# strasdat/ScaViSLAM

Measured on AMD Instinct MI355X. Metric: stereo frames/sec + DWO Schur ms @ 50 KF / 20k pts, higher is better.
Workload: dtype u8/int32 (FAST, ZNSSD), f32+f64 (dense tracking), f64 (Schur); 1 GPU

## Files before the change

scavislam_amd/csrc/motion.hip:

```cpp
#include "common.h"
#include "gate.h"
#include "lm6.h"
#include <algorithm>

namespace {

__device__ __forceinline__ void cloud_TQ(const double (&T)[12], const svs_cam &cam, double (&TQ)[16]) {
  double Ti[12];
#pragma unroll
  for (int r = 0; r < 3; ++r)
#pragma unroll
    for (int c = 0; c < 3; ++c) Ti[4 * r + c] = T[4 * c + r];
#pragma unroll
  for (int r = 0; r < 3; ++r) Ti[4 * r + 3] = -(Ti[4 * r] * T[3] + Ti[4 * r + 1] * T[7] + Ti[4 * r + 2] * T[11]);
  const double Q[16] = {1, 0, 0, -cam.cx, 0, 1, 0, -cam.cy, 0, 0, 0, cam.f, 0, 0, 1.0 / cam.b, 0};
#pragma unroll
  for (int r = 0; r < 4; ++r)
#pragma unroll
    for (int c = 0; c < 4; ++c) {
      double s = 0;
#pragma unroll
      for (int k = 0; k < 4; ++k) { double tik = r < 3 ? Ti[4 * r + k] : (k == 3 ? 1.0 : 0.0); s += tik * Q[4 * k + c]; }
      TQ[4 * r + c] = s;
    }
}
__device__ __forceinline__ void cloud_sample(const float *__restrict__ disp, int ds, int cw, int level, const double (&TQ)[16], int i, float *__restrict__ cloud) {
  const int u = i % cw, v = i / cw;
  const double inv_factor = 1.0 / (double)(1 << level);
  const float d = (float)(disp[(size_t)((v * 4) << level) * ds + ((u * 4) << level)] * inv_factor);
  float4 o;
  if (d <= 0) o = make_float4(0.f, 0.f, 0.f, -1.f);
  else {
    const double q[4] = {(double)(u * 4), (double)(v * 4), (double)d, 1.0};
    double r[4];
#pragma unroll
    for (int k = 0; k < 4; ++k) r[k] = TQ[4 * k] * q[0] + TQ[4 * k + 1] * q[1] + TQ[4 * k + 2] * q[2] + TQ[4 * k + 3] * q[3];
    o = make_float4((float)(r[0] / r[3]), (float)(r[1] / r[3]), (float)(r[2] / r[3]), 1.f);
  }
  reinterpret_cast<float4 *>(cloud)[i] = o;
}
__global__ __launch_bounds__(256) void pointcloud_cpu_sem_kernel(const float *__restrict__ disp, int ds, size_t disp_b, svs_cam cam,
                                                                 int level, const double *__restrict__ Tarr,
                                                                 float *__restrict__ cloud, size_t cloud_b) {
  const int slot = blockIdx.y;
  const int cw = cam.w / 4, ch = cam.h / 4;
  const int i = blockIdx.x * 256 + threadIdx.x;
  if (i >= cw * ch) return;
  double T[12], TQ[16];
#pragma unroll
  for (int k = 0; k < 12; ++k) T[k] = Tarr[(size_t)slot * 12 + k];
  cloud_TQ(T, cam, TQ);
  cloud_sample(disp + slot * disp_b, ds, cw, level, TQ, i, cloud + slot * cloud_b);
}

struct CloudLevels { svs_cam cam[3]; float *cloud[3]; size_t cloud_b[3]; int blocks[3]; };
__global__ __launch_bounds__(256) void pointcloud_cpu_sem_levels_kernel(const float *__restrict__ disp, int ds, size_t disp_b, CloudLevels Q, const double *__restrict__ Tarr) {
  const int slot = blockIdx.y;
  int bx = blockIdx.x, level = 0;
  if (bx >= Q.blocks[0]) { bx -= Q.blocks[0]; level = 1; if (bx >= Q.blocks[1]) { bx -= Q.blocks[1]; level = 2; } }
  const svs_cam cam = level == 0 ? Q.cam[0] : (level == 1 ? Q.cam[1] : Q.cam[2]);
  float *cloud = level == 0 ? Q.cloud[0] : (level == 1 ? Q.cloud[1] : Q.cloud[2]);
  const size_t cloud_b = level == 0 ? Q.cloud_b[0] : (level == 1 ? Q.cloud_b[1] : Q.cloud_b[2]);
  const int cw = cam.w / 4, ch = cam.h / 4;
  const int i = bx * 256 + threadIdx.x;
  if (i >= cw * ch) return;
  double T[12], TQ[16];
#pragma unroll
  for (int k = 0; k < 12; ++k) T[k] = Tarr[(size_t)slot * 12 + k];
  cloud_TQ(T, cam, TQ);
  cloud_sample(disp + slot * disp_b, ds, cw, level, TQ, i, cloud + slot * cloud_b);
}

}

int svs_pointcloud_cpu_sem_levels(svs_ctx *ctx, const float *d_disp, int disp_stride, size_t disp_bstride, const svs_cam *cams, const double *d_T, float *const *d_cloud,
                                  const size_t *cloud_bstride, int batch) {
  SVS_REQUIRE(ctx, ctx && d_disp && cams && d_T && d_cloud && cloud_bstride && batch >= 1);
  SVS_DEVICE(ctx);
  CloudLevels Q;
  int total = 0;
  for (int l = 0; l < 3; ++l) {
    SVS_REQUIRE(ctx, cams[l].w % 4 == 0 && cams[l].h % 4 == 0 && d_cloud[l]);
    Q.cam[l] = cams[l]; Q.cloud[l] = d_cloud[l]; Q.cloud_b[l] = cloud_bstride[l];
    Q.blocks[l] = div_up((cams[l].w / 4) * (cams[l].h / 4), 256);
    total += Q.blocks[l];
  }
  hipLaunchKernelGGL(pointcloud_cpu_sem_levels_kernel, dim3(total, batch), dim3(256), 0, ctx->stream, d_disp, disp_stride, disp_bstride, Q, d_T);
  SVS_LAUNCH_CHECK(ctx);
  return SVS_OK;
}

extern "C" int svs_pointcloud_cpu_sem(svs_ctx *ctx, const float *d_disp, int disp_stride, size_t disp_bstride,
                                      const svs_cam *cam, int level, const double *d_T, float *d_cloud,
                                      size_t cloud_bstride, int batch) {
  SVS_REQUIRE(ctx, ctx && d_disp && cam && d_T && d_cloud && level >= 0 && level < 3 && batch >= 1);
  SVS_DEVICE(ctx);
  SVS_REQUIRE(ctx, cam->w % 4 == 0 && cam->h % 4 == 0);
  int n = (cam->w / 4) * (cam->h / 4);
  hipLaunchKernelGGL(pointcloud_cpu_sem_kernel, dim3(div_up(n, 256), batch), dim3(256), 0, ctx->stream, d_disp, disp_stride,
                     disp_bstride, *cam, level, d_T, d_cloud, cloud_bstride);
  SVS_LAUNCH_CHECK(ctx);
  return SVS_OK;
}

namespace {

__device__ __forceinline__ double mo_kernel(double delta, double b) {
  const double a = fabs(delta);
  return a < b ? delta * delta : 2 * b * a - b * b;
}
__device__ __forceinline__ double mo_weighted_sq(double *f, int robust, double b) {
  if (robust) {
    const double nrm = fmax(1e-10, sqrt(f[0] * f[0] + f[1] * f[1] + f[2] * f[2]));
    const double w = sqrt(mo_kernel(nrm, b)) / nrm;
    f[0] *= w; f[1] *= w; f[2] *= w;
  }
  return f[0] * f[0] + f[1] * f[1] + f[2] * f[2];
}

constexpr int MO_THREADS = 256;
template <int N>
__device__ __forceinline__ void mo_reduce(double (&v)[N], int n_sum, double *s_red) {
  const int lane = threadIdx.x & 63, wave = threadIdx.x >> 6;
#pragma unroll
  for (int k = 0; k < N; ++k) {
    double x = v[k];
#pragma unroll
    for (int o = 32; o > 0; o >>= 1) { const double y = __shfl_xor(x, o, 64); x = k < n_sum ? x + y : fmax(x, y); }
    if (lane == 0) s_red[wave * N + k] = x;
  }
  __syncthreads();
  if (threadIdx.x < N) {
    const int k = threadIdx.x;
    double x = s_red[k];
    for (int w = 1; w < MO_THREADS / 64; ++w) x = k < n_sum ? x + s_red[w * N + k] : fmax(x, s_red[w * N + k]);
    s_red[(MO_THREADS / 64) * N + k] = x;
  }
  __syncthreads();
#pragma unroll
  for (int k = 0; k < N; ++k) v[k] = s_red[(MO_THREADS / 64) * N + k];
  __syncthreads();
}

__global__ __launch_bounds__(MO_THREADS) void motion_only_kernel(const svs_match_result *__restrict__ res, int n, size_t res_bstride, svs_cam cam,
                                                                 svs_pose_opt_params prm, double *__restrict__ T_io, svs_pose_opt_stats *__restrict__ stats) {
  __shared__ double s_red[(MO_THREADS / 64 + 1) * 28];
  __shared__ double s_T[12], s_Tn[12], s_B[6];
  const int tid = threadIdx.x, slot = blockIdx.x;
  res += (size_t)slot * res_bstride;
  if (tid < 12) s_T[tid] = T_io[12 * slot + tid];
  __syncthreads();
  double chi2, max_err, mu, nu = 2;
  int num_obs;
  {
    double v[4] = {0, 0, 0, 0};
    for (int i = tid; i < n; i += MO_THREADS) {
      if (res[i].status != 0) continue;
      double f[3], J[18];
      mo_residual<true>(s_T, res[i], cam, f, J);
#pragma unroll
      for (int c = 0; c < 6; ++c) v[3] = fmax(v[3], fabs(J[c] * J[c] + J[6 + c] * J[6 + c] + J[12 + c] * J[12 + c]));
      v[0] += mo_weighted_sq(f, prm.robust_kernel, prm.kernel_param);
      v[1] += 1.0;
      v[2] = fmax(v[2], fmax(fabs(f[0]), fmax(fabs(f[1]), fabs(f[2]))));
    }
    mo_reduce<4>(v, 2, s_red);
    chi2 = v[0]; num_obs = (int)v[1]; max_err = v[2];
    mu = prm.initial_mu == -1 ? prm.tau * v[3] : prm.initial_mu;
  }
  const double initial_chi2 = chi2;
  int status = num_obs == 0 ? 1 : (num_obs < prm.min_obs ? 3 : 0), trial = 0;
  bool stop = status != 0;
  for (int ig = 0; ig < prm.num_iter && !stop; ++ig) {
    double rho = 0;
    do {
      double v[27];
#pragma unroll
      for (int k = 0; k < 27; ++k) v[k] = 0;
      for (int i = tid; i < n; i += MO_THREADS) {
        if (res[i].status != 0) continue;
        double f[3], J[18];
        mo_residual<true>(s_T, res[i], cam, f, J);
        mo_weighted_sq(f, prm.robust_kernel, prm.kernel_param);
        int k = 0;
#pragma unroll
        for (int r = 0; r < 6; ++r) {
#pragma unroll
          for (int c = r; c < 6; ++c) v[k++] += J[r] * J[c] + J[6 + r] * J[6 + c] + J[12 + r] * J[12 + c];
          v[21 + r] += J[r] * f[0] + J[6 + r] * f[1] + J[12 + r] * f[2];
        }
      }
      mo_reduce<27>(v, 27, s_red);
      if (tid == 0) {
        double A[36], B[6], delta[6];
        int k = 0;
        for (int r = 0; r < 6; ++r)
          for (int c = r; c < 6; ++c) { A[6 * r + c] = A[6 * c + r] = v[k++]; }
        for (int r = 0; r < 6; ++r) { A[7 * r] += mu; B[r] = -v[21 + r]; s_B[r] = B[r]; }
        d_solve6(A, B, delta);
        double Tn[12];
        d_se3_exp_mul(delta, s_T, Tn);
        for (int i = 0; i < 12; ++i) s_Tn[i] = Tn[i];
      }
      __syncthreads();
      double w[2] = {0, 0};
      for (int i = tid; i < n; i += MO_THREADS) {
        if (res[i].status != 0) continue;
        double f[3];
        mo_residual<false>(s_Tn, res[i], cam, f, nullptr);
        w[0] += mo_weighted_sq(f, prm.robust_kernel, prm.kernel_param);
        w[1] = fmax(w[1], fmax(fabs(f[0]), fmax(fabs(f[1]), fabs(f[2]))));
      }
      mo_reduce<2>(w, 1, s_red);
      const double new_chi2 = w[0];
      if (isnan(new_chi2)) { status = 2; stop = true; break; }
      rho = chi2 - new_chi2;
      if (rho > 0) {
        if (tid < 12) s_T[tid] = s_Tn[tid];
        chi2 = new_chi2; max_err = w[1];
        double bm = -1;
        for (int c = 0; c < 6; ++c) bm = fmax(bm, fabs(s_B[c]));
        stop = bm <= 1e-10;
        const double q = 2 * rho - 1, sc = 1 - q * q * q;
        mu *= fmax(1. / 3., sc);
        nu = 2.; trial = 0;
      } else {
        mu *= nu; nu *= 2.; ++trial;
        if (trial == 5) stop = true;
      }
      __syncthreads();
    } while (!(rho > 0 || stop));
  }
  if (tid < 12) T_io[12 * slot + tid] = s_T[tid];
  if (tid == 0) {
    svs_pose_opt_stats st;
    st.initial_chi2 = initial_chi2; st.chi2 = chi2; st.max_err = max_err; st.num_obs = num_obs; st.status = status;
    stats[slot] = st;
  }
}

constexpr int MO2_THREADS = 256, MO2_RC = 6, MO2_WAVES = MO2_THREADS / 64;
struct MoObs { double o[3], q[3]; };

template <bool FIRST, bool JAC = true>
__device__ __forceinline__ void mo2_terms(const double (&T)[12], const MoObs &ob, const svs_cam &cam, int robust, double kb, double (&x)[32], double &max_err,
                                          double &max_diag) {
  static_assert(JAC || !FIRST, "the first sweep needs the Jacobian");
  const double *q = ob.q;
  const double X = T[0] * q[0] + T[1] * q[1] + T[2] * q[2] + T[3];
  const double Y = T[4] * q[0] + T[5] * q[1] + T[6] * q[2] + T[7];
  const double Z = T[8] * q[0] + T[9] * q[1] + T[10] * q[2] + T[11];
  const double fl = cam.f, iz = 1.0 / Z, fiz = fl * iz, Xb = X - cam.b;
  double f0 = ob.o[0] - (X * fiz + cam.cx), f1 = ob.o[1] - (Y * fiz + cam.cy), f2 = ob.o[2] - (Xb * fiz + cam.cx);
  const double A = -fiz, C = fiz * X * iz, D = fiz * Y * iz, E = fiz * Xb * iz;
  const double a3 = Y * C, a4 = Z * A - X * C, a5 = -Y * A;
  const double b3 = Y * D - Z * A, b4 = -X * D, b5 = X * A;
  const double c3 = Y * E, c4 = Z * A - X * E;
  if (FIRST) {
    const double AA = A * A;
    double m = fmax(AA + AA, AA);
    m = fmax(m, C * C + D * D + E * E);
    m = fmax(m, a3 * a3 + b3 * b3 + c3 * c3);
    m = fmax(m, a4 * a4 + b4 * b4 + c4 * c4);
    m = fmax(m, a5 * a5 + b5 * b5 + a5 * a5);
    max_diag = fmax(max_diag, m);
  }
  const double ss = f0 * f0 + f1 * f1 + f2 * f2;
  double chi = ss;
  if (robust) {
    const double nrm = fmax(1e-10, sqrt(ss));
    if (nrm >= kb) {
      const double k = 2 * kb * nrm - kb * kb, w = sqrt(k) / nrm;
      f0 *= w; f1 *= w; f2 *= w;
      chi = f0 * f0 + f1 * f1 + f2 * f2;
    }
  }
  x[27] += chi;
  max_err = fmax(max_err, fmax(fabs(f0), fmax(fabs(f1), fabs(f2))));
  if constexpr (!JAC) return;
  x[0] += A * A + A * A;          x[1] += 0.0;                     x[2] += A * C + A * E;
  x[3] += A * a3 + A * c3;        x[4] += A * a4 + A * c4;         x[5] += A * a5 + A * a5;
  x[6] += A * A;                  x[7] += A * D;                   x[8] += A * b3;
  x[9] += A * b4;                 x[10] += A * b5;
  x[11] += C * C + D * D + E * E; x[12] += C * a3 + D * b3 + E * c3; x[13] += C * a4 + D * b4 + E * c4;
  x[14] += C * a5 + D * b5 + E * a5;
  x[15] += a3 * a3 + b3 * b3 + c3 * c3; x[16] += a3 * a4 + b3 * b4 + c3 * c4; x[17] += a3 * a5 + b3 * b5 + c3 * a5;
  x[18] += a4 * a4 + b4 * b4 + c4 * c4; x[19] += a4 * a5 + b4 * b5 + c4 * a5;
  x[20] += a5 * a5 + b5 * b5 + a5 * a5;
  x[21] += A * f0 + A * f2;       x[22] += A * f1;                 x[23] += C * f0 + D * f1 + E * f2;
  x[24] += a3 * f0 + b3 * f1 + c3 * f2; x[25] += a4 * f0 + b4 * f1 + c4 * f2; x[26] += a5 * f0 + b5 * f1 + a5 * f2;
}
__device__ __forceinline__ int mo2_id(int lane) { return ((lane & 1) << 4) | ((lane & 2) << 2) | (lane & 4) | ((lane & 8) >> 2) | ((lane & 16) >> 4); }
__device__ __forceinline__ double mo2_wave_reduce(double (&x)[32]) {
  const int lane = threadIdx.x & 63;
#pragma unroll
  for (int step = 0; step < 5; ++step) {
    const int half = 16 >> step, bit = 1 << step;
    const bool up = (lane & bit) != 0;
#pragma unroll
    for (int k = 0; k < half; ++k) {
      double lo = x[k], hi = x[k + half];
      asm volatile("" : "+v"(lo), "+v"(hi));
      const double send = up ? lo : hi;
      const double keep = up ? hi : lo;
      x[k] = keep + __shfl_xor(send, bit, 64);
    }
  }
  return x[0] + __shfl_xor(x[0], 32, 64);
}

template <bool FIRST>
__device__ __forceinline__ void mo2_sweep(const double (&T)[12], const MoObs (&ob)[MO2_RC], int n_ok, const int *s_idx, const svs_match_result *__restrict__ res,
                                          const svs_cam &cam, int robust, double kb, double (*s_part)[32]) {
  const int tid = threadIdx.x, lane = tid & 63, wave = tid >> 6;
  double x[32];
#pragma unroll
  for (int i = 0; i < 32; ++i) x[i] = 0.0;
  double me = 0.0, md = 0.0;
#pragma unroll
  for (int k = 0; k < MO2_RC; ++k)
    if (tid + k * MO2_THREADS < n_ok) mo2_terms<FIRST>(T, ob[k], cam, robust, kb, x, me, md);
  for (int j = tid + MO2_RC * MO2_THREADS; j < n_ok; j += MO2_THREADS) {
    const svs_match_result &r = res[s_idx[j]];
    MoObs t;
#pragma unroll
    for (int c = 0; c < 3; ++c) { t.o[c] = r.obs[c]; t.q[c] = r.xyz_actkey[c]; }
    mo2_terms<FIRST>(T, t, cam, robust, kb, x, me, md);
  }
  const double v = mo2_wave_reduce(x);
#pragma unroll
  for (int o = 32; o > 0; o >>= 1) { me = fmax(me, __shfl_xor(me, o, 64)); if (FIRST) md = fmax(md, __shfl_xor(md, o, 64)); }
  const int id = mo2_id(lane);
  if (lane < 32 && id < 28) s_part[wave][id] = v;
  if (lane == 0) { s_part[wave][28] = me; s_part[wave][29] = md; }
}

__device__ __forceinline__ void mo2_sweep_chi2(const double (&T)[12], const MoObs (&ob)[MO2_RC], int n_ok, const int *s_idx, const svs_match_result *__restrict__ res,
                                               const svs_cam &cam, int robust, double kb, double (*s_part)[32]) {
  const int tid = threadIdx.x, lane = tid & 63, wave = tid >> 6;
  double x[32];
  x[27] = 0.0;
  double me = 0.0, md = 0.0;
#pragma unroll
  for (int k = 0; k < MO2_RC; ++k)
    if (tid + k * MO2_THREADS < n_ok) mo2_terms<false, false>(T, ob[k], cam, robust, kb, x, me, md);
  for (int j = tid + MO2_RC * MO2_THREADS; j < n_ok; j += MO2_THREADS) {
    const svs_match_result &r = res[s_idx[j]];
    MoObs t;
#pragma unroll
    for (int c = 0; c < 3; ++c) { t.o[c] = r.obs[c]; t.q[c] = r.xyz_actkey[c]; }
    mo2_terms<false, false>(T, t, cam, robust, kb, x, me, md);
  }
  double v = x[27];
#pragma unroll
  for (int o = 1; o <= 32; o <<= 1) v += __shfl_xor(v, o, 64);
#pragma unroll
  for (int o = 32; o > 0; o >>= 1) me = fmax(me, __shfl_xor(me, o, 64));
  if (lane == 0) { s_part[wave][27] = v; s_part[wave][28] = me; }
}

__device__ __forceinline__ void gate_stream(const svs_match_result *__restrict__ res, const svs_candidate_point *__restrict__ pts, int n, int n_new, const svs_cam &cam,
                                            const double (&T)[12], float mre, svs_gated_point *__restrict__ out, svs_point_stats *__restrict__ st, int tid, int *s_cnt,
                                            double *s_sum) {
  if (tid < 18) s_cnt[tid] = 0;
  __syncthreads();
  const int half_w = (int)(cam.w * 0.5), half_h = (int)(cam.h * 0.5);
  const float third = (float)(1. / 3.);
  const int third_w = (int)(cam.w * third), third_h = (int)(cam.h * third);
  const int tt_w = (int)(cam.w * 2 * third), tt_h = (int)(cam.h * 2 * third);
  double len = 0;
  for (int i = tid; i < n && tid < 256; i += 256) {
    svs_gated_point g{};
    if (res[i].status == 0) {
      atomicAdd(&s_cnt[17], 1);
      double d[3];
      mo_residual<false>(T, res[i], cam, d, nullptr);
      const int level = pts[i].anchor_level;
      const int factor = 1 << level;
      if (SVS_GATE_PASSES(d, factor, mre)) {
        const double *uvu = res[i].obs, *q = res[i].xyz_actkey;
        const int i2 = uvu[0] < half_w ? 0 : 1, j2 = uvu[1] < half_h ? 0 : 1;
        const int i3 = uvu[0] < third_w ? 0 : (uvu[0] < tt_w ? 1 : 2), j3 = uvu[1] < third_h ? 0 : (uvu[1] < tt_h ? 1 : 2);
        atomicAdd(&s_cnt[i2 * 2 + j2], 1);
        atomicAdd(&s_cnt[4 + i3 * 3 + j3], 1);
        atomicAdd(&s_cnt[13 + level], 1);
        atomicAdd(&s_cnt[16], 1);
        const double inv = 1.0 / (double)factor;
        g.accepted = 1;
        g.is_new = i < n_new ? 1 : 0;
        g.uv_pyr[0] = uvu[0] * inv; g.uv_pyr[1] = uvu[1] * inv;
        g.curkey_uv_pyr[0] = (q[0] / q[2] * cam.f + cam.cx) * inv;
        g.curkey_uv_pyr[1] = (q[1] / q[2] * cam.f + cam.cy) * inv;
        const double dx = g.uv_pyr[0] - g.curkey_uv_pyr[0], dy = g.uv_pyr[1] - g.curkey_uv_pyr[1];
        len += sqrt(dx * dx + dy * dy);
      }
    }
    out[i] = g;
  }
#pragma unroll
  for (int o = 32; o > 0; o >>= 1) len += __shfl_xor(len, o, 64);
  if ((tid & 63) == 0 && tid < 256) s_sum[tid >> 6] = len;
  __syncthreads();
  if (tid < 4) st->num_points_grid2x2[tid] = s_cnt[tid];
  else if (tid < 13) st->num_points_grid3x3[tid - 4] = s_cnt[tid];
  else if (tid < 16) st->num_matched_points[tid - 13] = s_cnt[tid];
  else if (tid == 16) st->num_track_points = s_cnt[16];
  else if (tid == 17) st->num_obs = s_cnt[17];
  else if (tid == 18) { st->pad_[0] = st->pad_[1] = 0; st->sum_track_length = (s_sum[0] + s_sum[1]) + (s_sum[2] + s_sum[3]); }
}
using MoTail = svs_mo_tail;
template <bool TAIL>
__global__ __launch_bounds__(MO2_THREADS) void motion_only_fused_kernel(const svs_match_result *__restrict__ res, int n, size_t res_bstride, svs_cam cam,
                                                                        svs_pose_opt_params prm, double *__restrict__ T_io,
                                                                        svs_pose_opt_stats *__restrict__ stats, MoTail Q, int spec) {
  extern __shared__ int s_idx[];
  __shared__ double s_part[MO2_WAVES][32];
  __shared__ double s_Tn[12], s_Tc[12];
  __shared__ int s_wcnt[8][MO2_WAVES];
  __shared__ int s_conv;
  const int tid = threadIdx.x, lane = tid & 63, wave = tid >> 6, slot = TAIL && Q.order ? (Q.order[blockIdx.x] >> 4) : (int)blockIdx.x;
  res += (size_t)slot * res_bstride;
  int n_ok = 0;
  for (int base = 0; base < n; base += 8 * MO2_THREADS) {
    int st[8];
#pragma unroll
    for (int c = 0; c < 8; ++c) { const int i = base + c * MO2_THREADS + tid; st[c] = i < n ? res[i].status : 1; }
    unsigned long long m[8];
#pragma unroll
    for (int c = 0; c < 8; ++c) { m[c] = __ballot(st[c] == 0); if (lane == 0) s_wcnt[c][wave] = __popcll(m[c]); }
    __syncthreads();
#pragma unroll
    for (int c = 0; c < 8; ++c) {
      int off = n_ok, tot = 0;
#pragma unroll
      for (int w = 0; w < MO2_WAVES; ++w) { const int k = s_wcnt[c][w]; off += w < wave ? k : 0; tot += k; }
      if (st[c] == 0) s_idx[off + __popcll(m[c] & ((1ull << lane) - 1ull))] = base + c * MO2_THREADS + tid;
      n_ok += tot;
    }
    __syncthreads();
  }
  MoObs ob[MO2_RC];
#pragma unroll
  for (int k = 0; k < MO2_RC; ++k) {
    const int j = tid + k * MO2_THREADS;
    if (j < n_ok) {
      const svs_match_result &r = res[s_idx[j]];
#pragma unroll
      for (int c = 0; c < 3; ++c) { ob[k].o[c] = r.obs[c]; ob[k].q[c] = r.xyz_actkey[c]; }
    }
  }
  auto total = [&](int id) { double s = s_part[0][id]; for (int w = 1; w < MO2_WAVES; ++w) s += s_part[w][id]; return s; };
  auto total_max = [&](int id) { double s = s_part[0][id]; for (int w = 1; w < MO2_WAVES; ++w) s = fmax(s, s_part[w][id]); return s; };
  auto uniform_pose = [&](const double *p, double (&T)[12]) {
#pragma unroll
    for (int i = 0; i < 12; ++i) {
      const double v = p[i];
      T[i] = __hiloint2double(__builtin_amdgcn_readfirstlane(__double2hiint(v)), __builtin_amdgcn_readfirstlane(__double2loint(v)));
    }
  };
  double Tn[12];
  uniform_pose(T_io + 12 * slot, Tn);
  if (tid < 12) s_Tc[tid] = T_io[12 * slot + tid];
  mo2_sweep<true>(Tn, ob, n_ok, s_idx, res, cam, prm.robust_kernel, prm.kernel_param, s_part);
  __syncthreads();
  const int num_obs = n_ok;
  double chi2 = total(27), max_err = total_max(28), mu = prm.initial_mu == -1 ? prm.tau * total_max(29) : prm.initial_mu, nu = 2;
  const double initial_chi2 = chi2;
  int status = num_obs == 0 ? 1 : (num_obs < prm.min_obs ? 3 : 0), trial = 0;
  bool stop = status != 0;
  double col[6] = {0, 0, 0, 0, 0, 0};
  auto load_system = [&]() {
    if (wave == 0 && lane < 7) {
#pragma unroll
      for (int r = 0; r < 6; ++r) {
        const int a = r < lane ? r : lane, b = r < lane ? lane : r;
        col[r] = lane < 6 ? total(a * (13 - a) / 2 + (b - a)) : -total(21 + r);
      }
    }
  };
  load_system();
  for (int ig = 0; ig < prm.num_iter && !stop; ++ig) {
    double rho = 0;
    do {
      if (wave == 0) {
        double a[6], bmax = 0, delta[6];
#pragma unroll
        for (int r = 0; r < 6; ++r) a[r] = col[r] + (r == lane ? mu : 0.0);
#pragma unroll
        for (int r = 0; r < 6; ++r) bmax = fmax(bmax, fabs(mo2_bcast(col[r], 6)));
        wave_solve6(a, delta);
        double Tc[12], Tx[12];
#pragma unroll
        for (int i = 0; i < 12; ++i) Tc[i] = s_Tc[i];
        mo2_exp_mul(delta, Tc, Tx);
        if (lane < 12) {
          double v = Tx[0];
#pragma unroll
          for (int i = 1; i < 12; ++i) v = lane == i ? Tx[i] : v;
          s_Tn[lane] = v;
        }
        if (lane == 0) s_conv = bmax <= 1e-10 ? 1 : 0;
      }
      __syncthreads();
      uniform_pose(s_Tn, Tn);
      const int conv = s_conv;
      const bool lean = spec != 0 && trial >= 1;
      if (lean) mo2_sweep_chi2(Tn, ob, n_ok, s_idx, res, cam, prm.robust_kernel, prm.kernel_param, s_part);
      else mo2_sweep<false>(Tn, ob, n_ok, s_idx, res, cam, prm.robust_kernel, prm.kernel_param, s_part);
      __syncthreads();
      const double new_chi2 = total(27), new_max = total_max(28);
      if (isnan(new_chi2)) { status = 2; stop = true; break; }
      rho = chi2 - new_chi2;
      if (rho > 0 && lean) {
        __syncthreads();
        mo2_sweep<false>(Tn, ob, n_ok, s_idx, res, cam, prm.robust_kernel, prm.kernel_param, s_part);
        __syncthreads();
      }
      if (rho > 0) {
        if (tid < 12) s_Tc[tid] = s_Tn[tid];
        chi2 = new_chi2; max_err = new_max;
        load_system();
        stop = conv != 0;
        const double q = 2 * rho - 1, sc = 1 - q * q * q;
        mu *= fmax(1. / 3., sc);
        nu = 2.; trial = 0;
      } else {
        mu *= nu; nu *= 2.; ++trial;
        if (trial == 5) stop = true;
      }
    } while (!(rho > 0 || stop));
  }
  if (tid < 12) T_io[12 * slot + tid] = s_Tc[tid];
  if (tid == 0) {
    svs_pose_opt_stats st;
    st.initial_chi2 = initial_chi2; st.chi2 = chi2; st.max_err = max_err; st.num_obs = num_obs; st.status = status;
    stats[slot] = st;
  }
  if constexpr (TAIL) {
    __shared__ int s_gcnt[18];
    __shared__ double s_gsum[4];
    __syncthreads();
    double T[12];
#pragma unroll
    for (int i = 0; i < 12; ++i) T[i] = s_Tc[i];
    gate_stream(res, Q.pts + slot * Q.pts_b, n, Q.n_new[slot], cam, T, Q.mre, Q.gated + slot * Q.gated_b, Q.ptstats + slot, tid, s_gcnt, s_gsum);
#pragma unroll 1
    for (int l = 0; l < 3; ++l) {
      double TQ[16];
      cloud_TQ(T, Q.cams[l], TQ);
      const int cw = Q.cams[l].w / 4, n_px = cw * (Q.cams[l].h / 4);
      const float *disp = Q.disp + slot * Q.disp_b;
      float *cloud = Q.cloud[l] + slot * Q.cloud_b[l];
      for (int i = tid; i < n_px; i += MO2_THREADS) cloud_sample(disp, Q.ds, cw, l, TQ, i, cloud);
    }
  }
}

}
namespace {
__global__ __launch_bounds__(256) void gate_matched_kernel(const svs_match_result *__restrict__ res, const svs_candidate_point *__restrict__ pts, int n,
                                                           size_t res_b, size_t pts_b, int n_new, const int32_t *__restrict__ n_new_arr, svs_cam cam,
                                                           const double *__restrict__ Tarr, float mre, svs_gated_point *__restrict__ out, size_t out_b,
                                                           svs_point_stats *__restrict__ stats) {
  __shared__ int s_cnt[18];
  __shared__ double s_sum[4];
  const int tid = threadIdx.x, slot = blockIdx.x;
  if (n_new_arr) n_new = n_new_arr[slot];
  double T[12];
#pragma unroll
  for (int k = 0; k < 12; ++k) T[k] = Tarr[12 * slot + k];
  gate_stream(res + slot * res_b, pts + slot * pts_b, n, n_new, cam, T, mre, out + slot * out_b, stats + slot, tid, s_cnt, s_sum);
}
}

extern "C" int svs_process_matched_points(svs_ctx *ctx, const svs_match_result *d_results, const svs_candidate_point *d_pts, int n,
                                          size_t res_bstride, size_t pts_bstride, int n_new_records, const svs_cam *cam, const double *d_T,
                                          float max_reproj_error, svs_gated_point *d_gated, size_t gated_bstride, svs_point_stats *d_stats,
                                          int batch) {
  SVS_REQUIRE(ctx, ctx && cam && d_T && d_stats && batch >= 1 && n >= 0 && (n == 0 || (d_results && d_pts && d_gated)));
  SVS_DEVICE(ctx);
  hipLaunchKernelGGL(gate_matched_kernel, dim3(batch), dim3(256), 0, ctx->stream, d_results, d_pts, n, res_bstride, pts_bstride, n_new_records,
                     (const int32_t *)nullptr, *cam, d_T, max_reproj_error, d_gated, gated_bstride, d_stats);
  SVS_LAUNCH_CHECK(ctx);
  return SVS_OK;
}
int svs_process_matched_points_dev(svs_ctx *ctx, const svs_match_result *d_results, const svs_candidate_point *d_pts, int n, size_t res_bstride,
                                   size_t pts_bstride, const int32_t *d_n_new_records, const svs_cam *cam, const double *d_T, float max_reproj_error,
                                   svs_gated_point *d_gated, size_t gated_bstride, svs_point_stats *d_stats, int batch) {
  SVS_REQUIRE(ctx, ctx && cam && d_T && d_stats && d_n_new_records && batch >= 1 && n >= 0 && (n == 0 || (d_results && d_pts && d_gated)));
  SVS_DEVICE(ctx);
  hipLaunchKernelGGL(gate_matched_kernel, dim3(batch), dim3(256), 0, ctx->stream, d_results, d_pts, n, res_bstride, pts_bstride, 0, d_n_new_records, *cam, d_T,
                     max_reproj_error, d_gated, gated_bstride, d_stats);
  SVS_LAUNCH_CHECK(ctx);
  return SVS_OK;
}

int svs_motion_only_gate_cloud(svs_ctx *ctx, const svs_match_result *d_results, int n, size_t res_bstride, const svs_cam *cam, const svs_pose_opt_params *prm,
                               double *d_T_io, svs_pose_opt_stats *d_stats, const svs_mo_tail *tail, int batch) {
  SVS_REQUIRE(ctx, ctx && cam && prm && d_T_io && d_stats && tail && batch >= 1 && n >= 1 && d_results);
  SVS_DEVICE(ctx);
  if ((size_t)n * sizeof(int) > 48 * 1024 || ctx->mo_legacy) return SVS_ERR_UNSUPPORTED;
  for (int l = 0; l < 3; ++l) SVS_REQUIRE(ctx, tail->cams[l].w % 4 == 0 && tail->cams[l].h % 4 == 0 && tail->cloud[l]);
  hipLaunchKernelGGL(motion_only_fused_kernel<true>, dim3(batch), dim3(MO2_THREADS), (size_t)n * sizeof(int), ctx->stream, d_results, n, res_bstride, *cam, *prm, d_T_io,
                     d_stats, *tail, ctx->mo_spec);
  SVS_LAUNCH_CHECK(ctx);
  return SVS_OK;
}

extern "C" int svs_motion_only(svs_ctx *ctx, const svs_match_result *d_results, int n, size_t res_bstride, const svs_cam *cam,
                               const svs_pose_opt_params *prm, double *d_T_io, svs_pose_opt_stats *d_stats, int batch) {
  SVS_REQUIRE(ctx, ctx && cam && prm && d_T_io && d_stats && batch >= 1 && n >= 0 && (n == 0 || d_results));
  SVS_DEVICE(ctx);
  if ((size_t)n * sizeof(int) <= 48 * 1024 && !ctx->mo_legacy)
    hipLaunchKernelGGL(motion_only_fused_kernel<false>, dim3(batch), dim3(MO2_THREADS), (size_t)std::max(n, 1) * sizeof(int), ctx->stream, d_results, n, res_bstride, *cam,
                       *prm, d_T_io, d_stats, MoTail{}, ctx->mo_spec);
  else
    hipLaunchKernelGGL(motion_only_kernel, dim3(batch), dim3(MO_THREADS), 0, ctx->stream, d_results, n, res_bstride, *cam, *prm, d_T_io, d_stats);
  SVS_LAUNCH_CHECK(ctx);
  return SVS_OK;
}
```

Measured before the change: 218,700 frames/s.

## Stage overflow observations in LDS and batch loads in gate and cloud loops

Observations beyond the six register-cached ones per thread are now staged once into shared memory, up to 512 of them. Each LM sweep then reads them from LDS instead of re-gathering them through the index list from global memory. The gating loop and the point-cloud tail loop are restructured to issue several independent global loads (8 and 16 per lane) before computing, which exposes memory-level parallelism. The status-scan load is also clamped so it is unconditional. The changes raise the LDS footprint and register pressure, which may lower occupancy, and the cloud loop now does incremental u/v stepping.

```diff
diff --git a/scavislam_amd/csrc/motion.hip b/scavislam_amd/csrc/motion.hip
--- a/scavislam_amd/csrc/motion.hip
+++ b/scavislam_amd/csrc/motion.hip
@@ -24,10 +24,10 @@
       TQ[4 * r + c] = s;
     }
 }
-__device__ __forceinline__ void cloud_sample(const float *__restrict__ disp, int ds, int cw, int level, const double (&TQ)[16], int i, float *__restrict__ cloud) {
-  const int u = i % cw, v = i / cw;
+__device__ __forceinline__ size_t cloud_disp_offset(int ds, int level, int u, int v) { return (size_t)((v * 4) << level) * ds + ((u * 4) << level); }
+__device__ __forceinline__ float4 cloud_point(float raw, int level, const double (&TQ)[16], int u, int v) {
   const double inv_factor = 1.0 / (double)(1 << level);
-  const float d = (float)(disp[(size_t)((v * 4) << level) * ds + ((u * 4) << level)] * inv_factor);
+  const float d = (float)(raw * inv_factor);
   float4 o;
   if (d <= 0) o = make_float4(0.f, 0.f, 0.f, -1.f);
   else {
@@ -37,7 +37,34 @@
     for (int k = 0; k < 4; ++k) r[k] = TQ[4 * k] * q[0] + TQ[4 * k + 1] * q[1] + TQ[4 * k + 2] * q[2] + TQ[4 * k + 3] * q[3];
     o = make_float4((float)(r[0] / r[3]), (float)(r[1] / r[3]), (float)(r[2] / r[3]), 1.f);
   }
-  reinterpret_cast<float4 *>(cloud)[i] = o;
+  return o;
+}
+__device__ __forceinline__ void cloud_sample(const float *__restrict__ disp, int ds, int cw, int level, const double (&TQ)[16], int i, float *__restrict__ cloud) {
+  const int u = i % cw, v = i / cw;
+  reinterpret_cast<float4 *>(cloud)[i] = cloud_point(disp[cloud_disp_offset(ds, level, u, v)], level, TQ, u, v);
+}
+template <int U, int LANES>
+__device__ __forceinline__ void cloud_samples_strided(const float *__restrict__ disp, int ds, int cw, int n_px, int level, const double (&TQ)[16], int first,
+                                                      float *__restrict__ cloud) {
+  const int du = LANES % cw, dv = LANES / cw;
+  int u = first % cw, v = first / cw;
+  for (int i = first; i < n_px; i += U * LANES) {
+    float raw[U];
+    int ul = u, vl = v;
+#pragma unroll
+    for (int g = 0; g < U; ++g) {
+      const bool in = i + g * LANES < n_px;
+      raw[g] = disp[cloud_disp_offset(ds, level, in ? ul : 0, in ? vl : 0)];
+      ul += du; vl += dv;
+      if (ul >= cw) { ul -= cw; ++vl; }
+    }
+#pragma unroll
+    for (int g = 0; g < U; ++g) {
+      if (i + g * LANES < n_px) reinterpret_cast<float4 *>(cloud)[i + g * LANES] = cloud_point(raw[g], level, TQ, u, v);
+      u += du; v += dv;
+      if (u >= cw) { u -= cw; ++v; }
+    }
+  }
 }
 __global__ __launch_bounds__(256) void pointcloud_cpu_sem_kernel(const float *__restrict__ disp, int ds, size_t disp_b, svs_cam cam,
                                                                  int level, const double *__restrict__ Tarr,
@@ -241,6 +268,12 @@
 
 constexpr int MO2_THREADS = 256, MO2_RC = 6, MO2_WAVES = MO2_THREADS / 64;
 struct MoObs { double o[3], q[3]; };
+constexpr int MO2_OV = 512, MO2_OV_MAX_N = 9216;
+__host__ __device__ inline int mo2_ov_cap(int n) { return n > MO2_RC * MO2_THREADS && n <= MO2_OV_MAX_N ? MO2_OV : 0; }
+__host__ __device__ inline int mo2_idx_words(int n) { return ((n > 1 ? n : 1) + 3) & ~3; }
+inline size_t mo2_lds_bytes(int n) { return (size_t)mo2_idx_words(n) * sizeof(int) + (size_t)mo2_ov_cap(n) * sizeof(MoObs); }
+static_assert(MO2_OV % MO2_THREADS == 0, "a lane owns whole columns of the overflow");
+static_assert(MO2_OV_MAX_N * sizeof(int) + MO2_OV * sizeof(MoObs) + 2048 <= 64 * 1024, "index list + overflow + the kernel's static LDS (1.5 KB) within a workgroup's 64 KB");
 
 template <bool FIRST, bool JAC = true>
 __device__ __forceinline__ void mo2_terms(const double (&T)[12], const MoObs &ob, const svs_cam &cam, int robust, double kb, double (&x)[32], double &max_err,
@@ -310,7 +343,7 @@
 }
 
 template <bool FIRST>
-__device__ __forceinline__ void mo2_sweep(const double (&T)[12], const MoObs (&ob)[MO2_RC], int n_ok, const int *s_idx, const svs_match_result *__restrict__ res,
+__device__ __forceinline__ void mo2_sweep(const double (&T)[12], const MoObs (&ob)[MO2_RC], int n_ok, const int *s_idx, const MoObs *s_ov, int ov_cap, const svs_match_result *__restrict__ res,
                                           const svs_cam &cam, int robust, double kb, double (*s_part)[32]) {
   const int tid = threadIdx.x, lane = tid & 63, wave = tid >> 6;
   double x[32];
@@ -320,7 +353,10 @@
 #pragma unroll
   for (int k = 0; k < MO2_RC; ++k)
     if (tid + k * MO2_THREADS < n_ok) mo2_terms<FIRST>(T, ob[k], cam, robust, kb, x, me, md);
-  for (int j = tid + MO2_RC * MO2_THREADS; j < n_ok; j += MO2_THREADS) {
+#pragma unroll
+  for (int k = 0; k < MO2_OV / MO2_THREADS; ++k)
+    if (k * MO2_THREADS < ov_cap && tid + (MO2_RC + k) * MO2_THREADS < n_ok) mo2_terms<FIRST>(T, s_ov[tid + k * MO2_THREADS], cam, robust, kb, x, me, md);
+  for (int j = tid + MO2_RC * MO2_THREADS + ov_cap; j < n_ok; j += MO2_THREADS) {
     const svs_match_result &r = res[s_idx[j]];
     MoObs t;
 #pragma unroll
@@ -335,7 +371,7 @@
   if (lane == 0) { s_part[wave][28] = me; s_part[wave][29] = md; }
 }
 
-__device__ __forceinline__ void mo2_sweep_chi2(const double (&T)[12], const MoObs (&ob)[MO2_RC], int n_ok, const int *s_idx, const svs_match_result *__restrict__ res,
+__device__ __forceinline__ void mo2_sweep_chi2(const double (&T)[12], const MoObs (&ob)[MO2_RC], int n_ok, const int *s_idx, const MoObs *s_ov, int ov_cap, const svs_match_result *__restrict__ res,
                                                const svs_cam &cam, int robust, double kb, double (*s_part)[32]) {
   const int tid = threadIdx.x, lane = tid & 63, wave = tid >> 6;
   double x[32];
@@ -344,7 +380,10 @@
 #pragma unroll
   for (int k = 0; k < MO2_RC; ++k)
     if (tid + k * MO2_THREADS < n_ok) mo2_terms<false, false>(T, ob[k], cam, robust, kb, x, me, md);
-  for (int j = tid + MO2_RC * MO2_THREADS; j < n_ok; j += MO2_THREADS) {
+#pragma unroll
+  for (int k = 0; k < MO2_OV / MO2_THREADS; ++k)
+    if (k * MO2_THREADS < ov_cap && tid + (MO2_RC + k) * MO2_THREADS < n_ok) mo2_terms<false, false>(T, s_ov[tid + k * MO2_THREADS], cam, robust, kb, x, me, md);
+  for (int j = tid + MO2_RC * MO2_THREADS + ov_cap; j < n_ok; j += MO2_THREADS) {
     const svs_match_result &r = res[s_idx[j]];
     MoObs t;
 #pragma unroll
@@ -359,6 +398,7 @@
   if (lane == 0) { s_part[wave][27] = v; s_part[wave][28] = me; }
 }
 
+constexpr int GATE_G = 8;
 __device__ __forceinline__ void gate_stream(const svs_match_result *__restrict__ res, const svs_candidate_point *__restrict__ pts, int n, int n_new, const svs_cam &cam,
                                             const double (&T)[12], float mre, svs_gated_point *__restrict__ out, svs_point_stats *__restrict__ st, int tid, int *s_cnt,
                                             double *s_sum) {
@@ -369,33 +409,54 @@
   const int third_w = (int)(cam.w * third), third_h = (int)(cam.h * third);
   const int tt_w = (int)(cam.w * 2 * third), tt_h = (int)(cam.h * 2 * third);
   double len = 0;
-  for (int i = tid; i < n && tid < 256; i += 256) {
-    svs_gated_point g{};
-    if (res[i].status == 0) {
-      atomicAdd(&s_cnt[17], 1);
-      double d[3];
-      mo_residual<false>(T, res[i], cam, d, nullptr);
-      const int level = pts[i].anchor_level;
-      const int factor = 1 << level;
-      if (SVS_GATE_PASSES(d, factor, mre)) {
-        const double *uvu = res[i].obs, *q = res[i].xyz_actkey;
-        const int i2 = uvu[0] < half_w ? 0 : 1, j2 = uvu[1] < half_h ? 0 : 1;
-        const int i3 = uvu[0] < third_w ? 0 : (uvu[0] < tt_w ? 1 : 2), j3 = uvu[1] < third_h ? 0 : (uvu[1] < tt_h ? 1 : 2);
-        atomicAdd(&s_cnt[i2 * 2 + j2], 1);
-        atomicAdd(&s_cnt[4 + i3 * 3 + j3], 1);
-        atomicAdd(&s_cnt[13 + level], 1);
-        atomicAdd(&s_cnt[16], 1);
-        const double inv = 1.0 / (double)factor;
-        g.accepted = 1;
-        g.is_new = i < n_new ? 1 : 0;
-        g.uv_pyr[0] = uvu[0] * inv; g.uv_pyr[1] = uvu[1] * inv;
-        g.curkey_uv_pyr[0] = (q[0] / q[2] * cam.f + cam.cx) * inv;
-        g.curkey_uv_pyr[1] = (q[1] / q[2] * cam.f + cam.cy) * inv;
-        const double dx = g.uv_pyr[0] - g.curkey_uv_pyr[0], dy = g.uv_pyr[1] - g.curkey_uv_pyr[1];
-        len += sqrt(dx * dx + dy * dy);
-      }
-    }
-    out[i] = g;
+  for (int i0 = tid; i0 < n && tid < 256; i0 += GATE_G * 256) {
+    svs_match_result r[GATE_G];
+    int lvl[GATE_G];
+#pragma unroll
+    for (int k = 0; k < GATE_G; ++k) {
+      const int i = i0 + k * 256, ic = i < n ? i : n - 1;
+      r[k].status = res[ic].status;
+#pragma unroll
+      for (int c = 0; c < 3; ++c) { r[k].obs[c] = res[ic].obs[c]; r[k].xyz_actkey[c] = res[ic].xyz_actkey[c]; }
+      lvl[k] = pts[ic].anchor_level;
+    }
+#pragma unroll
+    for (int k = 0; k < GATE_G; ++k) {
+      asm volatile("" : "+v"(r[k].status), "+v"(lvl[k]));
+#pragma unroll
+      for (int c = 0; c < 3; ++c) asm volatile("" : "+v"(r[k].obs[c]), "+v"(r[k].xyz_actkey[c]));
+    }
+#pragma unroll
+    for (int k = 0; k < GATE_G; ++k) {
+      const int i = i0 + k * 256;
+      if (i >= n) continue;
+      svs_gated_point g{};
+      if (r[k].status == 0) {
+        atomicAdd(&s_cnt[17], 1);
+        double d[3];
+        mo_residual<false>(T, r[k], cam, d, nullptr);
+        const int level = lvl[k];
+        const int factor = 1 << level;
+        if (SVS_GATE_PASSES(d, factor, mre)) {
+          const double *uvu = r[k].obs, *q = r[k].xyz_actkey;
+          const int i2 = uvu[0] < half_w ? 0 : 1, j2 = uvu[1] < half_h ? 0 : 1;
+          const int i3 = uvu[0] < third_w ? 0 : (uvu[0] < tt_w ? 1 : 2), j3 = uvu[1] < third_h ? 0 : (uvu[1] < tt_h ? 1 : 2);
+          atomicAdd(&s_cnt[i2 * 2 + j2], 1);
+          atomicAdd(&s_cnt[4 + i3 * 3 + j3], 1);
+          atomicAdd(&s_cnt[13 + level], 1);
+          atomicAdd(&s_cnt[16], 1);
+          const double inv = 1.0 / (double)factor;
+          g.accepted = 1;
+          g.is_new = i < n_new ? 1 : 0;
+          g.uv_pyr[0] = uvu[0] * inv; g.uv_pyr[1] = uvu[1] * inv;
+          g.curkey_uv_pyr[0] = (q[0] / q[2] * cam.f + cam.cx) * inv;
+          g.curkey_uv_pyr[1] = (q[1] / q[2] * cam.f + cam.cy) * inv;
+          const double dx = g.uv_pyr[0] - g.curkey_uv_pyr[0], dy = g.uv_pyr[1] - g.curkey_uv_pyr[1];
+          len += sqrt(dx * dx + dy * dy);
+        }
+      }
+      out[i] = g;
+    }
   }
 #pragma unroll
   for (int o = 32; o > 0; o >>= 1) len += __shfl_xor(len, o, 64);
@@ -409,22 +470,29 @@
   else if (tid == 18) { st->pad_[0] = st->pad_[1] = 0; st->sum_track_length = (s_sum[0] + s_sum[1]) + (s_sum[2] + s_sum[3]); }
 }
 using MoTail = svs_mo_tail;
+constexpr int CLOUD_U = 16;
 template <bool TAIL>
 __global__ __launch_bounds__(MO2_THREADS) void motion_only_fused_kernel(const svs_match_result *__restrict__ res, int n, size_t res_bstride, svs_cam cam,
                                                                         svs_pose_opt_params prm, double *__restrict__ T_io,
                                                                         svs_pose_opt_stats *__restrict__ stats, MoTail Q, int spec) {
-  extern __shared__ int s_idx[];
+  extern __shared__ __align__(16) int s_idx[];
   __shared__ double s_part[MO2_WAVES][32];
   __shared__ double s_Tn[12], s_Tc[12];
   __shared__ int s_wcnt[8][MO2_WAVES];
   __shared__ int s_conv;
   const int tid = threadIdx.x, lane = tid & 63, wave = tid >> 6, slot = TAIL && Q.order ? (Q.order[blockIdx.x] >> 4) : (int)blockIdx.x;
   res += (size_t)slot * res_bstride;
+  const int ov_cap = mo2_ov_cap(n);
+  MoObs *s_ov = reinterpret_cast<MoObs *>(s_idx + mo2_idx_words(n));
   int n_ok = 0;
   for (int base = 0; base < n; base += 8 * MO2_THREADS) {
     int st[8];
 #pragma unroll
-    for (int c = 0; c < 8; ++c) { const int i = base + c * MO2_THREADS + tid; st[c] = i < n ? res[i].status : 1; }
+    for (int c = 0; c < 8; ++c) {
+      const int i = base + c * MO2_THREADS + tid;
+      const int s = res[i < n ? i : n - 1].status;
+      st[c] = i < n ? s : 1;
+    }
     unsigned long long m[8];
 #pragma unroll
     for (int c = 0; c < 8; ++c) { m[c] = __ballot(st[c] == 0); if (lane == 0) s_wcnt[c][wave] = __popcll(m[c]); }
@@ -449,6 +517,21 @@
       for (int c = 0; c < 3; ++c) { ob[k].o[c] = r.obs[c]; ob[k].q[c] = r.xyz_actkey[c]; }
     }
   }
+  {
+    MoObs t[MO2_OV / MO2_THREADS];
+#pragma unroll
+    for (int k = 0; k < MO2_OV / MO2_THREADS; ++k) {
+      const int j = tid + (MO2_RC + k) * MO2_THREADS;
+      if (k * MO2_THREADS < ov_cap && j < n_ok) {
+        const svs_match_result &r = res[s_idx[j]];
+#pragma unroll
+        for (int c = 0; c < 3; ++c) { t[k].o[c] = r.obs[c]; t[k].q[c] = r.xyz_actkey[c]; }
+      }
+    }
+#pragma unroll
+    for (int k = 0; k < MO2_OV / MO2_THREADS; ++k)
+      if (k * MO2_THREADS < ov_cap && tid + (MO2_RC + k) * MO2_THREADS < n_ok) s_ov[tid + k * MO2_THREADS] = t[k];
+  }
   auto total = [&](int id) { double s = s_part[0][id]; for (int w = 1; w < MO2_WAVES; ++w) s += s_part[w][id]; return s; };
   auto total_max = [&](int id) { double s = s_part[0][id]; for (int w = 1; w < MO2_WAVES; ++w) s = fmax(s, s_part[w][id]); return s; };
   auto uniform_pose = [&](const double *p, double (&T)[12]) {
@@ -461,7 +544,7 @@
   double Tn[12];
   uniform_pose(T_io + 12 * slot, Tn);
   if (tid < 12) s_Tc[tid] = T_io[12 * slot + tid];
-  mo2_sweep<true>(Tn, ob, n_ok, s_idx, res, cam, prm.robust_kernel, prm.kernel_param, s_part);
+  mo2_sweep<true>(Tn, ob, n_ok, s_idx, s_ov, ov_cap, res, cam, prm.robust_kernel, prm.kernel_param, s_part);
   __syncthreads();
   const int num_obs = n_ok;
   double chi2 = total(27), max_err = total_max(28), mu = prm.initial_mu == -1 ? prm.tau * total_max(29) : prm.initial_mu, nu = 2;
@@ -505,15 +588,15 @@
       uniform_pose(s_Tn, Tn);
       const int conv = s_conv;
       const bool lean = spec != 0 && trial >= 1;
-      if (lean) mo2_sweep_chi2(Tn, ob, n_ok, s_idx, res, cam, prm.robust_kernel, prm.kernel_param, s_part);
-      else mo2_sweep<false>(Tn, ob, n_ok, s_idx, res, cam, prm.robust_kernel, prm.kernel_param, s_part);
+      if (lean) mo2_sweep_chi2(Tn, ob, n_ok, s_idx, s_ov, ov_cap, res, cam, prm.robust_kernel, prm.kernel_param, s_part);
+      else mo2_sweep<false>(Tn, ob, n_ok, s_idx, s_ov, ov_cap, res, cam, prm.robust_kernel, prm.kernel_param, s_part);
       __syncthreads();
       const double new_chi2 = total(27), new_max = total_max(28);
       if (isnan(new_chi2)) { status = 2; stop = true; break; }
       rho = chi2 - new_chi2;
       if (rho > 0 && lean) {
         __syncthreads();
-        mo2_sweep<false>(Tn, ob, n_ok, s_idx, res, cam, prm.robust_kernel, prm.kernel_param, s_part);
+        mo2_sweep<false>(Tn, ob, n_ok, s_idx, s_ov, ov_cap, res, cam, prm.robust_kernel, prm.kernel_param, s_part);
         __syncthreads();
       }
       if (rho > 0) {
@@ -551,7 +634,7 @@
       const int cw = Q.cams[l].w / 4, n_px = cw * (Q.cams[l].h / 4);
       const float *disp = Q.disp + slot * Q.disp_b;
       float *cloud = Q.cloud[l] + slot * Q.cloud_b[l];
-      for (int i = tid; i < n_px; i += MO2_THREADS) cloud_sample(disp, Q.ds, cw, l, TQ, i, cloud);
+      cloud_samples_strided<CLOUD_U, MO2_THREADS>(disp, Q.ds, cw, n_px, l, TQ, tid, cloud);
     }
   }
 }
@@ -601,7 +684,7 @@
   SVS_DEVICE(ctx);
   if ((size_t)n * sizeof(int) > 48 * 1024 || ctx->mo_legacy) return SVS_ERR_UNSUPPORTED;
   for (int l = 0; l < 3; ++l) SVS_REQUIRE(ctx, tail->cams[l].w % 4 == 0 && tail->cams[l].h % 4 == 0 && tail->cloud[l]);
-  hipLaunchKernelGGL(motion_only_fused_kernel<true>, dim3(batch), dim3(MO2_THREADS), (size_t)n * sizeof(int), ctx->stream, d_results, n, res_bstride, *cam, *prm, d_T_io,
+  hipLaunchKernelGGL(motion_only_fused_kernel<true>, dim3(batch), dim3(MO2_THREADS), mo2_lds_bytes(n), ctx->stream, d_results, n, res_bstride, *cam, *prm, d_T_io,
                      d_stats, *tail, ctx->mo_spec);
   SVS_LAUNCH_CHECK(ctx);
   return SVS_OK;
@@ -612,7 +695,7 @@
   SVS_REQUIRE(ctx, ctx && cam && prm && d_T_io && d_stats && batch >= 1 && n >= 0 && (n == 0 || d_results));
   SVS_DEVICE(ctx);
   if ((size_t)n * sizeof(int) <= 48 * 1024 && !ctx->mo_legacy)
-    hipLaunchKernelGGL(motion_only_fused_kernel<false>, dim3(batch), dim3(MO2_THREADS), (size_t)std::max(n, 1) * sizeof(int), ctx->stream, d_results, n, res_bstride, *cam,
+    hipLaunchKernelGGL(motion_only_fused_kernel<false>, dim3(batch), dim3(MO2_THREADS), mo2_lds_bytes(n), ctx->stream, d_results, n, res_bstride, *cam,
                        *prm, d_T_io, d_stats, MoTail{}, ctx->mo_spec);
   else
     hipLaunchKernelGGL(motion_only_kernel, dim3(batch), dim3(MO_THREADS), 0, ctx->stream, d_results, n, res_bstride, *cam, *prm, d_T_io, d_stats);
```

New measurement: 223,800 frames/s, median of 5. 2.3% higher.
